# StavrosOrf/EV2Gym

Hardware: AMD Instinct MI355X
Metric: env-steps/sec (envs x chargers x steps); % HBM roofline (higher is better)
Workload: dtype f64; 1 GPU; cfg2: V2GProfitPlusLoads, 50 chargers, 1 transformer, uniform[-1,1] actions; envs_per_gpu=4096, scenario_pool_per_gpu=32768, scenario_pool_order=sorted by busy window inside every window of envs_per_gpu scenarios, chargers=50, transformers=1, steps_per_episode=112, obs_dim=162, soc_log=True, launch=persistent, actor=none

## Files before the change

### ev2gym_amd/csrc/ev2g_device.h

```cpp
#pragma once
#include <hip/hip_runtime.h>
#include <stdint.h>

#define EV2G_BLOCK 256
#define EV2G_NQ 8

struct __attribute__((aligned(128))) SessRec {
    double pacmax, ts;
    double tsm, eta_ch;
    double gate_ch;
    double B;
    double rB;
    double v;
    double rv;
    double gate_dis;
    double minB, emerg;
    double pdismax, eta_dis;
    double cap0;
    double potc;
};
struct SessTail {
    double des;
    int nt_arr, nt_dep;
};
// ... 825 lines not shown
            }
        }
        t += 1;
        __syncthreads();
    }
}

__global__ void ev2g_build_window_table_kernel(DevScn s, double *__restrict__ tab, int m0, int m1) {
    const long long per = (long long)s.R * (s.T + 1) * 40, n = per * m1;
    for (long long i = per * m0 + blockIdx.x * (long long)blockDim.x + threadIdx.x; i < n; i += (long long)gridDim.x * blockDim.x) {
        const int j = (int)(i % 40);
        const long long k = i / 40;
        const int step = (int)(k % (s.T + 1));
        const int er = (int)(k / (s.T + 1));
        tab[i] = (j < 20) ? load_minus_pv_at(s, (long long)er * s.T, step, j) : power_limit_at(s, er, step, j - 20);
    }
}

__global__ void ev2g_build_head_table_kernel(const double *__restrict__ price_ch, const double *__restrict__ win_tab,
                                             int m0, int m1, int T, int NH, double *__restrict__ tab) {
    const long long per = (long long)(T + 1) * NH, n = per * m1;
    for (long long i = per * m0 + blockIdx.x * (long long)blockDim.x + threadIdx.x; i < n; i += (long long)gridDim.x * blockDim.x) {
        const int c = (int)(i % NH);
        const long long row = i / NH;
        const int step = (int)(row % (T + 1));
        const long long e = row / (T + 1);
        double v;
        if (c < 20) { const int k = step + c; v = (k < T) ? fabs(price_ch[e * T + k]) : 0.0; }
        else v = win_tab[row * 40 + (c - 20)];
        tab[i] = v;
    }
}

__global__ void ev2g_build_step_table_kernel(DevScn s, double *__restrict__ tab, int m0, int m1) {
    const long long n = (long long)m1 * s.T;
    for (long long i = (long long)m0 * s.T + blockIdx.x * (long long)blockDim.x + threadIdx.x; i < n; i += (long long)gridDim.x * blockDim.x) {
        double *o = tab + i * 8;
        o[0] = s.price_ch[i]; o[1] = s.price_dis[i]; o[2] = s.tr_base[i]; o[3] = s.tr_maxp[i]; o[4] = s.tr_minp[i];
        o[5] = s.setpoint[i]; o[6] = 0.0; o[7] = 0.0;
    }
}

__global__ void __launch_bounds__(64) ev2g_build_occ_mask_kernel(DevScn s, double *__restrict__ step_tab, int m0, int m1) {
    const int lane = threadIdx.x, P = s.P, T = s.T;
    for (int m = m0 + blockIdx.x; m < m1; m += gridDim.x) {
        int ta = EV2G_INT_MAX, td = -1, ss = -1;
        if (lane < P) {
            const long long gs = (long long)m * P + lane;
            const int2 w = s.port_first_win[gs];
            ta = w.x; td = w.y; ss = s.port_first[gs];
        }
        for (int t = 0; t < T; t++) {
            const bool occ = (ta <= t) && (t <= td);
            if (occ && t >= td) {
                const SessTail tl = s.tail[ss];
                ta = tl.nt_arr; td = tl.nt_dep;
                ss = (ta != EV2G_INT_MAX) ? ss + 1 : -1;
            }
            const unsigned long long m_occ = __ballot(occ), m_arr = __ballot(ta == t + 1);
            if (lane == 0) {
                double *o = step_tab + ((long long)m * T + t) * 8;
                o[6] = __longlong_as_double((long long)m_occ); o[7] = __longlong_as_double((long long)m_arr);
            }
        }
    }
}

__host__ __device__ inline double ev2g_u01(uint64_t seed, uint64_t i) {
    uint64_t z = seed + 0x9E3779B97F4A7C15ull * (i + 1);
    z = (z ^ (z >> 30)) * 0xBF58476D1CE4E5B9ull;
    z = (z ^ (z >> 27)) * 0x94D049BB133111EBull;
    z = z ^ (z >> 31);
    return (double)(z >> 11) * (1.0 / 9007199254740992.0);
}

__global__ void ev2g_fill_uniform_kernel(double *dst, long long n, uint64_t seed, double lo, double hi) {
    for (long long i = blockIdx.x * (long long)blockDim.x + threadIdx.x; i < n; i += (long long)gridDim.x * blockDim.x)
        dst[i] = lo + (hi - lo) * ev2g_u01(seed, (uint64_t)i);
}

__device__ __forceinline__ double wave_sum(double v) {
    for (int d = 32; d > 0; d >>= 1) v += __shfl_xor(v, d, 64);
    return v;
}
__device__ __forceinline__ double wave_min(double v) {
    for (int d = 32; d > 0; d >>= 1) v = fmin(v, __shfl_xor(v, d, 64));
    return v;
}

__device__ __forceinline__ void port_sessions(const DevScn &s, const DevState &st, long long g, long long gs, int cur_step, int &first,
                                              int &last, bool &attached) {
    first = s.port_first[gs];
    last = first;
    attached = false;
    if (first < 0) return;
    const int2 w = make_int2(st.line[g].ta, st.line[g].td);
    const int cur = st.line[g].ss;
    if (cur < 0) {
        last = s.port_end[gs];
    } else {
        attached = (w.x <= cur_step);
        last = attached ? cur + 1 : cur;
    }
}

template <int EPWS> __device__ __forceinline__ double seg_sum(double v) {
    v += xor1_f64(v);
    v += xor2_f64(v);
    v += xor4_f64(v);
    v += dpp_mov_f64<0x128>(v);
    const int lo = __double2loint(v), hi = __double2hiint(v);
    const double r0 = __hiloint2double(__builtin_amdgcn_readlane(hi, 0), __builtin_amdgcn_readlane(lo, 0));
    const double r1 = __hiloint2double(__builtin_amdgcn_readlane(hi, 16), __builtin_amdgcn_readlane(lo, 16));
    const double r2 = __hiloint2double(__builtin_amdgcn_readlane(hi, 32), __builtin_amdgcn_readlane(lo, 32));
    const double r3 = __hiloint2double(__builtin_amdgcn_readlane(hi, 48), __builtin_amdgcn_readlane(lo, 48));
    if (EPWS == 1) return (r0 + r1) + (r2 + r3);
    return (threadIdx.x < 32) ? r0 + r1 : r2 + r3;
}
template <int EPWS> __device__ __forceinline__ double seg_min(double v) {
    v = fmin(v, xor1_f64(v));
    v = fmin(v, xor2_f64(v));
    v = fmin(v, xor4_f64(v));
    v = fmin(v, dpp_mov_f64<0x128>(v));
    const int lo = __double2loint(v), hi = __double2hiint(v);
    const double r0 = __hiloint2double(__builtin_amdgcn_readlane(hi, 0), __builtin_amdgcn_readlane(lo, 0));
    const double r1 = __hiloint2double(__builtin_amdgcn_readlane(hi, 16), __builtin_amdgcn_readlane(lo, 16));
    const double r2 = __hiloint2double(__builtin_amdgcn_readlane(hi, 32), __builtin_amdgcn_readlane(lo, 32));
    const double r3 = __hiloint2double(__builtin_amdgcn_readlane(hi, 48), __builtin_amdgcn_readlane(lo, 48));
    if (EPWS == 1) return fmin(fmin(r0, r1), fmin(r2, r3));
    return (threadIdx.x < 32) ? fmin(r0, r1) : fmin(r2, r3);
}
template <int EPWS> __device__ __forceinline__ bool seg_all(bool p) {
    const unsigned long long m = __ballot(p);
    if (EPWS == 1) return m == ~0ull;
    return (threadIdx.x < 32) ? ((unsigned)m == 0xffffffffu) : ((unsigned)(m >> 32) == 0xffffffffu);
}

struct StatsView {
    int T, C, R, P, dt;
    const double *setpoint;
    const int *scn_sess, *scn_sess_end, *ss_slot, *ss_tarr, *ss_tdep;
    const double *ss_B, *ss_afap;
    const int *cs_served;
    const double *cs_sat_sum, *hist, *env_acc, *sess_final_cap, *sess_abs_e, *soc_log;
    const PortLine *line;
};
__device__ __forceinline__ StatsView ev2g_stats_view(const DevScn &s, const DevState &st, const double *ss_afap) {
    return StatsView{s.T, s.C, s.R, s.P, s.dt, s.setpoint, s.scn_sess, s.scn_sess_end, s.ss_slot, s.ss_tarr, s.ss_tdep, s.ss_B, ss_afap,
                     st.cs_served, st.cs_sat_sum, st.hist, st.env_acc, st.sess_final_cap, st.sess_abs_e, st.soc_log, st.line};
}

#define EV2G_STATS_NK 40
#define EV2G_STATS_TB 8
#define EV2G_STATS_LK 16

template <int EPWS, int NK, int LK>
__device__ __forceinline__ void ev2g_env_stats(const StatsView &sv, int e, bool e_valid, int scn, int lane, int cur_step, double *__restrict__ out,
                                               double *l_keep, int lslot) {
    constexpr int W = 64 / EPWS;
    const int T = sv.T, C = sv.C, R = sv.R, P = sv.P;
    double served = 0.0, sat = 0.0, nsat = 0.0;
    for (int c = lane; c < C; c += W) {
        const int n = sv.cs_served[(long long)e * C + c];
        served += n;
        if (n > 0) { sat += sv.cs_sat_sum[(long long)e * C + c] / n; nsat += 1.0; }
    }
    served = seg_sum<EPWS>(served); sat = seg_sum<EPWS>(sat); nsat = seg_sum<EPWS>(nsat);
    double over = 0.0, te = 0.0, ete = 0.0, ptv = 0.0;
    for (int t = lane; t < T; t += W) {
        const bool past = t < cur_step;
        if (past) for (int r = 0; r < R; r++) over += sv.hist[EV2G_HIST(e, t, T, R) + 2 + r];
        const double sp = sv.setpoint[(long long)scn * T + t], u = past ? sv.hist[EV2G_HIST(e, t, T, R)] : 0.0;
        const double d = sp - u;
        te += d * d;
        ete += fabs(d);
        if (u > sp) ptv += u - sp;
    }
    over = seg_sum<EPWS>(over); te = seg_sum<EPWS>(te); ete = seg_sum<EPWS>(ete); ptv = seg_sum<EPWS>(ptv);
    ete *= (double)sv.dt / 60.0;
    if (lane == 0 && e_valid) {
        double *o = out + (long long)e * 17;
        o[0] = served;
        o[4] = (nsat > 0.0) ? sat / nsat : NAN;
        o[5] = ptv;
        o[6] = te;
        o[7] = ete;
        o[12] = over;
    }
    const double e0 = 7.543e6, e1 = 23.75e6, e2 = 6976, z0 = 7.348e-3, z1 = 3.667, z2 = 7.6e-4, z3 = 4.081e-3;
    const double b_cap_ah = 2.05, b_cap_kwh = 78, d_dist = 15000, b_age = 2 * 365, G_ = 0.186;
    const double theta = 298.15, kk = 0.8263, v_min = 3.3324;
    const double k_arrh = exp(-e2 / theta), k_age = pow(b_age, 0.25);
    const double Q_acc = 2 * (b_age * (d_dist / 365) * G_ * b_cap_ah) / b_cap_kwh, k_qacc = pow(Q_acc, 0.5);
    const bool log_soc = sv.soc_log != nullptr;
    double sum = 0.0, mn = INFINITY, cnt = 0.0, deg_cal = 0.0, deg_cyc = 0.0;
    double vkeep[2];
    int nkeep = 0;
    const int d0 = sv.scn_sess[scn], d1 = sv.scn_sess_end[scn];
    for (int k0 = d0; k0 < d1; k0 += W) {
        const int k = min(k0 + lane, d1 - 1);
        const bool has = k0 + lane < d1;
        const int q = sv.ss_slot[k], ta = sv.ss_tarr[k], td = sv.ss_tdep[k];
        const double B = sv.ss_B[k], afap = sv.ss_afap[k], fin_cap = sv.sess_final_cap[k];
        const double fin_abs = log_soc ? sv.sess_abs_e[k] : 0.0;
        const long long g = (long long)e * P + q;
        const bool spawned = has && ta <= cur_step;
        const bool live = td >= cur_step;
        const double l_cap = sv.line[g].cap, l_abs = sv.line[g].abse;
        const double capk = live ? l_cap : fin_cap;
        if (spawned) {
            const double v = capk / afap * 100.0;
            sum += v;
            mn = fmin(mn, v);
            cnt += 1.0;
            if (nkeep < 2) vkeep[nkeep] = v;
            nkeep++;
        }
        if (spawned) {
            if (log_soc) {
                const double *__restrict__ slog = sv.soc_log + (long long)e * T * P + q;
                const int tend = min(td, cur_step - 1);
                const double soc_f = capk / B;
                const double invB = 1.0 / B;
                double hs = 0.0, fs = 0.0;
                int n = 0, nf = 0;
                double xk[NK];
#pragma unroll
                for (int u = 0; u < NK; u++) xk[u] = slog[(long long)min(ta + u, tend) * P];
#pragma unroll
                for (int u = 0; u < NK; u++) {
                    if (ta + u <= tend) {
                        const double soc = fabs(xk[u]) * invB;
                        hs += soc; n++;
                        if (__double_as_longlong(xk[u]) >= 0) { fs += soc; nf++; }
                    }
                }
                for (int t = ta + NK; t <= tend; t += EV2G_STATS_TB) {
                    double x[EV2G_STATS_TB];
#pragma unroll
                    for (int u = 0; u < EV2G_STATS_TB; u++) x[u] = slog[(long long)min(t + u, tend) * P];
                    if (LK > 0 && t - ta - NK < LK) {
#pragma unroll
                        for (int u = 0; u < EV2G_STATS_TB; u++) l_keep[(t - ta - NK + u) * 64 + lslot] = x[u];
                    }
#pragma unroll
                    for (int u = 0; u < EV2G_STATS_TB; u++) {
                        if (t + u <= tend) {
                            const double soc = fabs(x[u]) * invB;
                            hs += soc; n++;
                            if (__double_as_longlong(x[u]) >= 0) { fs += soc; nf++; }
                        }
                    }
                }
                hs += soc_f; n++;
                fs += soc_f; nf++;
                const double avg_soc = hs / n, avg_f = fs / nf;
                double mad = 0.0;
#pragma unroll
                for (int u = 0; u < NK; u++)
                    if (ta + u <= tend && __double_as_longlong(xk[u]) >= 0) mad += fabs(avg_f - fabs(xk[u]) * invB);
                for (int t = ta + NK; t <= tend; t += EV2G_STATS_TB) {
                    double x[EV2G_STATS_TB];
                    if (LK > 0 && t - ta - NK < LK) {
#pragma unroll
                        for (int u = 0; u < EV2G_STATS_TB; u++) x[u] = l_keep[(t - ta - NK + u) * 64 + lslot];
                    } else {
#pragma unroll
                        for (int u = 0; u < EV2G_STATS_TB; u++) x[u] = slog[(long long)min(t + u, tend) * P];
                    }
#pragma unroll
                    for (int u = 0; u < EV2G_STATS_TB; u++)
                        if (t + u <= tend && __double_as_longlong(x[u]) >= 0) mad += fabs(avg_f - fabs(x[u]) * invB);
                }
                mad += fabs(avg_f - soc_f);
                const double delta_DoD = 2 * (mad / nf);
                const double T_sim = (td - ta + 1) * (double)sv.dt / (60 * 24);
                const double v_avg = v_min + kk * avg_soc;
                const double alpha = (e0 * v_avg - e1) * k_arrh;
                deg_cal += alpha * 0.75 * T_sim / k_age;
                const double v_half = v_min + kk * 0.5;
                const double beta = z0 * (v_half - z1) * (v_half - z1) + z2 + z3 * delta_DoD;
                const double abs_e = live ? l_abs : fin_abs;
                const double Q_sim = (abs_e / b_cap_kwh) * b_cap_ah;
                deg_cyc += beta * 0.5 * Q_sim / k_qacc;
            }
        }
    }
    sum = seg_sum<EPWS>(sum); cnt = seg_sum<EPWS>(cnt); mn = seg_min<EPWS>(mn);
    deg_cal = seg_sum<EPWS>(deg_cal); deg_cyc = seg_sum<EPWS>(deg_cyc);
    if (lane == 0 && e_valid) {
        const double *acc = sv.env_acc + (long long)e * 8;
        double *o = out + (long long)e * 17;
        o[1] = acc[1];
        o[2] = acc[2];
        o[3] = acc[3];
        o[11] = acc[4];
        o[13] = log_soc ? deg_cal + deg_cyc : NAN;
        o[14] = log_soc ? deg_cal : NAN;
        o[15] = log_soc ? deg_cyc : NAN;
        o[16] = acc[0];
    }
    double mean = NAN, sd = NAN, mnv = NAN;
    if (cnt > 0.0) {
        mean = sum / cnt;
        double var = 0.0;
        if (seg_all<EPWS>(nkeep <= 2)) {
            if (nkeep > 0) { const double v = vkeep[0] - mean; var += v * v; }
            if (nkeep > 1) { const double v = vkeep[1] - mean; var += v * v; }
        } else {
            for (int k = d0 + lane; k < d1; k += W) {
                const int ta = sv.ss_tarr[k];
                if (ta <= cur_step) {
                    const double capk = (sv.ss_tdep[k] >= cur_step) ? sv.line[(long long)e * P + sv.ss_slot[k]].cap : sv.sess_final_cap[k];
                    const double v = capk / sv.ss_afap[k] * 100.0 - mean;
                    var += v * v;
                }
            }
        }
        var = seg_sum<EPWS>(var);
        sd = sqrt(var / cnt);
        mnv = mn;
    }
    if (lane == 0 && e_valid) {
        double *o = out + (long long)e * 17;
        o[8] = mean;
        o[9] = sd;
        o[10] = mnv;
    }
}

template <int W>
__device__ __forceinline__ void ev2g_env_reset(const DevScn &s, const DevState &st, int e, int lane, int reset_off, double *__restrict__ r_obs,
                                               float *__restrict__ r_obs32) {
    const int T = s.T, C = s.C, R = s.R, P = s.P;
    const int scn_n = ev2g_scn(e, reset_off, s.M);
    const bool hfast = s.head_tab != nullptr && s.state_kind != 1 && 2 + s.head_nh <= 2 * W && (r_obs || r_obs32);
    double hrow0 = 0.0, hrow1 = 0.0;
    if (hfast) {
        const double *row = s.head_tab + (long long)scn_n * (T + 1) * s.head_nh;
        hrow0 = row[min(max(lane - 2, 0), s.head_nh - 1)];
        hrow1 = row[min(lane + W - 2, s.head_nh - 1)];
    }
    for (int q = lane; q < P; q += W) {
        const long long g = (long long)e * P + q, gs = (long long)scn_n * P + q;
        const int2 w = s.port_first_win[gs];
        st.line[g].ta = w.x; st.line[g].td = w.y; st.line[g].ss = s.port_first[gs]; st.line[g].cyc_lut = 0;
        st.line[g].cap = 0.0; st.line[g].tot = 0.0; st.line[g].prev = 0.0;
        st.port_energy[g] = 0.0; st.port_current[g] = 0.0;
        if (r_obs) { double *o = r_obs + (long long)e * s.D + s.slot_obs[q]; o[0] = 0.0; o[1] = 0.0; if (s.state_kind == 1) o[2] = 0.0; }
        if (r_obs32) { float *o = r_obs32 + (long long)e * s.D + s.slot_obs[q]; o[0] = 0.f; o[1] = 0.f; if (s.state_kind == 1) o[2] = 0.f; }
    }
    for (int c = lane; c < C; c += W) {
        const long long gc = (long long)e * C + c;
        st.cs_sat_sum[gc] = 0.0; st.cs_served[gc] = 0;
        if (st.cs_profits) { st.cs_profits[gc] = 0.0; st.cs_e_ch[gc] = 0.0; st.cs_e_dis[gc] = 0.0; st.cs_power_now[gc] = 0.0; st.cs_cur_now[gc] = 0.0; }
    }
    for (int i = lane; i < 8; i += W) st.env_acc[(long long)e * 8 + i] = 0.0;
    if (lane == 0) st.hist[EV2G_HIST(e, 0, T, R) + 1] = 0.0;
    for (int r = lane; r < R; r += W) st.tr_power_now[(long long)e * R + r] = 0.0;
    if (lane == 0) st.env_fault[e] = 0;
    if (hfast) {
        const int c0 = lane, c1 = lane + W, nc = 2 + s.head_nh;
        const double v0 = (c0 < 2) ? 0.0 : hrow0;
        if (r_obs) { double *o = r_obs + (long long)e * s.D; if (c0 < nc) o[c0] = v0; if (c1 < nc) o[c1] = hrow1; }
        if (r_obs32) { float *o = r_obs32 + (long long)e * s.D; if (c0 < nc) o[c0] = (float)v0; if (c1 < nc) o[c1] = (float)hrow1; }
    } else {
        if (r_obs) write_obs_env(s, r_obs + (long long)e * s.D, scn_n, 0, 0.0, lane, W);
        if (r_obs32) write_obs_env(s, r_obs32 + (long long)e * s.D, scn_n, 0, 0.0, lane, W);
    }
}
// ... 28 lines not shown
```

### ev2gym_amd/csrc/ev2g_step_wave.h

```cpp
#pragma once
#include <type_traits>
#include "ev2g_step_v2.h"
#include "ev2g_mlp.h"

#define EV2G_WAVE_BLOCK 256

__host__ __device__ inline size_t ev2g_wave_lds_bytes(int envs_per_group, int block = EV2G_WAVE_BLOCK) {
    const size_t NS = (size_t)block;
    return sizeof(double) * (EV2G_NQ * (NS + 8) + 7 * NS + 7 * (size_t)envs_per_group + 4 * 64) + sizeof(int) * (6 * NS + 8);
}
#define EV2G_INL_STATS_NK 12
#define EV2G_INL_STATS_LK 16
__host__ __device__ inline size_t ev2g_inl_stats_lds_bytes(int block = EV2G_WAVE_BLOCK) { return (size_t)block * EV2G_INL_STATS_LK * sizeof(double); }
#define EV2G_FUSED_BLOCK 1024
#define EV2G_FUSED_SX 200
#define EV2G_FUSED_RING 10
#define EV2G_FUSED_RING2 7

#define EV2G_FUSED_SXF 196
#define EV2G_FUSED_RINGF 4
__host__ __device__ inline size_t ev2g_fused_lds_bytes(int envs_per_wave = 1, int weight_terms = 1) {
    if (weight_terms > 1)
        return ev2g_wave_lds_bytes(EV2G_FUSED_BLOCK / 64 * envs_per_wave, EV2G_FUSED_BLOCK) + (size_t)16 * EV2G_FUSED_SXF * 4;
    return ev2g_wave_lds_bytes(EV2G_FUSED_BLOCK / 64 * envs_per_wave, EV2G_FUSED_BLOCK) + (size_t)16 * EV2G_FUSED_SX * 2 + (size_t)(25 + 19 + 4) * 16 * 4;
}
struct FusedArgs {
    MlpDev m;
    const float *obs0;
};

typedef const char __attribute__((address_space(1))) *gcptr;
typedef char __attribute__((address_space(1))) *gptr;
template <class T, class B> __device__ __forceinline__ T ldg32(B base, unsigned boff) {
    return *(const T __attribute__((address_space(1))) *)((gcptr)base + boff);
}
template <class T, class B> __device__ __forceinline__ T ldg32_nt(B base, unsigned boff) {
    return __builtin_nontemporal_load((const T __attribute__((address_space(1))) *)((gcptr)base + boff));
}
template <class T, class B> __device__ __forceinline__ void stg32(B base, unsigned boff, T v) {
    *(T __attribute__((address_space(1))) *)((gptr)base + boff) = v;
}
template <class T, class B> __device__ __forceinline__ void stg32_nt(B base, unsigned boff, T v) {
    __builtin_nontemporal_store(v, (T __attribute__((address_space(1))) *)((gptr)base + boff));
}
typedef double d2v __attribute__((ext_vector_type(2)));
typedef double d2v_a8 __attribute__((ext_vector_type(2), aligned(8)));
typedef int i2v __attribute__((ext_vector_type(2)));
typedef int i4v __attribute__((ext_vector_type(4)));
typedef float f2v __attribute__((ext_vector_type(2)));
template <class B> __device__ __forceinline__ SessRec ldg32_rec_charge(B base, unsigned boff) {
    union { SessRec r; d2v v[sizeof(SessRec) / 16]; } u;
    static_assert(sizeof(SessRec) == 128 && offsetof(SessRec, rB) == 48 && offsetof(SessRec, rv) == 64 && offsetof(SessRec, minB) == 80 && offsetof(SessRec, cap0) == 112,
                  "charging reads chunks 0..4, discharging chunks 3..6");
#pragma unroll
    for (int i = 0; i < 5; i++) u.v[i] = ldg32<d2v>(base, boff + 16u * i);
    asm volatile("" : "+v"(u.v[0]), "+v"(u.v[1]), "+v"(u.v[2]), "+v"(u.v[3]), "+v"(u.v[4]));
    return u.r;
}
template <class B> __device__ __forceinline__ SessRec ldg32_rec_discharge(B base, unsigned boff) {
    union { SessRec r; d2v v[sizeof(SessRec) / 16]; } u;
#pragma unroll
    for (int i = 3; i < 7; i++) u.v[i] = ldg32<d2v>(base, boff + 16u * i);
    asm volatile("" : "+v"(u.v[3]), "+v"(u.v[4]), "+v"(u.v[5]), "+v"(u.v[6]));
    return u.r;
}

template <class B> __device__ __forceinline__ SessRec ldg32_cls_charge(B base, unsigned boff) {
    static_assert(sizeof(ClsRec) == 128 && offsetof(ClsRec, gate_ch) == 16 && offsetof(ClsRec, rB) == 32 && offsetof(ClsRec, rv) == 48 && offsetof(ClsRec, v_d) == 64 &&
                  offsetof(ClsRec, gate_dis) == 80 && offsetof(ClsRec, emerg) == 96, "ClsRec layout");
    d2v c[4];
#pragma unroll
    for (int i = 0; i < 4; i++) c[i] = ldg32<d2v>(base, boff + 16u * i);
    asm volatile("" : "+v"(c[0]), "+v"(c[1]), "+v"(c[2]), "+v"(c[3]));
    SessRec r;
    r.pacmax = c[0].x; r.tsm = c[0].y; r.gate_ch = c[1].x; r.B = c[1].y; r.rB = c[2].x; r.v = c[2].y; r.rv = c[3].x;
    return r;
}
template <class B> __device__ __forceinline__ SessRec ldg32_cls_discharge(B base, unsigned boff) {
    d2v c[3];
#pragma unroll
    for (int i = 0; i < 3; i++) c[i] = ldg32<d2v>(base, boff + 64u + 16u * i);
    asm volatile("" : "+v"(c[0]), "+v"(c[1]), "+v"(c[2]));
    SessRec r;
    r.v = c[0].x; r.rv = c[0].y; r.gate_dis = c[1].x; r.minB = c[1].y; r.emerg = c[2].x; r.pdismax = c[2].y;
    return r;
}

struct WaveArgs {
    int P, T, E, D, M;
    char *slab_port; unsigned long long slab_port_slice;
    double *hist;
    double *env_acc;
    const double *cs_pack;
    char *lines;
    const double *step_tab;
    char *port_dyn;
    int dict;
    int epw, es;
};

template <int SK, int RK, bool IO32, int FULLK = 0, int BLOCK = EV2G_WAVE_BLOCK, bool ACT = false, int AE = 1, int NWF = 1>
__global__ void __launch_bounds__(BLOCK, 4) ev2g_step_wave(const V2P *__restrict__ params, StepIO io, int t0,
                                                           int k_steps, int auto_reset, WaveArgs wa, FusedArgs fa) {
    extern __shared__ double lds[];
    static_assert(!ACT || (IO32 && FULLK == 2 && BLOCK == EV2G_FUSED_BLOCK), "the fused actor + step instantiation");
    static_assert(AE == 1 || (ACT && SK == 1 && AE == 2), "two envs per wavefront in the fused instantiation: PublicPST only");
    static_assert(NWF == 1 || (ACT && AE == 1 && NWF == 2), "the float32 policy inside the launch: one env per wavefront (16 policy rows per workgroup)");
    constexpr bool FULL = FULLK >= 1, WIDE = FULLK >= 2, STR = FULLK >= 3 || ACT;
    constexpr bool STR_NT = FULLK >= 3;
    constexpr bool F64 = FULL && !IO32, F32 = FULL && IO32;
    constexpr bool LSO = FULL && !STR;
    constexpr bool INL = FULLK == 2 && !IO32 && !ACT && BLOCK == EV2G_WAVE_BLOCK;
#if defined(EV2G_PHASE_TIMING) && defined(EV2G_PT_OUTER)
    const unsigned long long pt_k0 = __builtin_readcyclecounter();
#endif
    typedef const V2P __attribute__((address_space(4))) *ParamPtr;
    ParamPtr S = (ParamPtr)(unsigned long long)params;
    constexpr int NS = BLOCK;
    constexpr int RS = NS + 8;
    const int P = wa.P, T = wa.T, E = wa.E, D = wa.D, M = wa.M;
    int off = io.scn_off;
    const gptr slabP = (gptr)wa.slab_port, hist = (gptr)wa.hist, slabS = (gptr)S->slab_sess;
    const unsigned long long PS8 = wa.slab_port_slice, SS8 = S->sess_slice;
    const gptr env_acc = (gptr)wa.env_acc;
#define PA(k) (slabP + PS8 * (unsigned long long)(k))
    const int EPW = ACT ? AE : wa.epw;
    const int ES = ACT ? (AE == 1 ? P : 32) : wa.es;
    const int G = (BLOCK / 64) * EPW;
    int grp;
    {
        const int nb = gridDim.x, b = blockIdx.x, per = nb >> 3;
        grp = (nb & 7) == 0 ? (b & 7) * per + (b >> 3) : b;
    }
    const int e0 = grp * G;
    double *stage = lds;
    double *s_cap = stage + (size_t)EV2G_NQ * RS;
    double *s_tot = s_cap + NS, *s_prev = s_tot + NS, *s_bcap = s_prev + NS, *s_potc = s_bcap + NS;
    double *s_amps = s_potc + NS, *s_abse = s_amps + NS;
    double *eacc = s_abse + NS;
    double *s_cst = eacc + 7 * G;
    int *s_ta = (int *)(s_cst + 4 * 64);
    int *s_td = s_ta + NS, *s_ss = s_td + NS, *s_cyc = s_ss + NS, *s_dirty = s_cyc + NS, *items = s_dirty + NS;
    int *cnt = items + NS;
    double *s_ts = s_bcap, *s_etac = s_potc, *s_etad = (double *)s_ta;
    constexpr int LUTMASK = FULL ? 0xfff : 0xffff;
    typedef typename std::conditional<SK == 1, MlpS16<2, 25, 19, 2, 1, 4, AE>, MlpS16<6, 25, 19, 4, 1, 4, AE>>::type MC;
    constexpr int FSX = MC::SX;
    constexpr int FKS1 = (SK == 1) ? 2 : 6, FNT3 = (SK == 1) ? 2 : 4;
    uint16_t *bufX = (uint16_t *)(cnt + 8);
    float *lbias = (float *)(bufX + 16 * EV2G_FUSED_SX);
    float *act_lds = (float *)s_amps;
    uint16_t *bufH1 = (uint16_t *)stage, *bufH2 = bufH1 + 16 * AE * MC::SH1;
    constexpr int FSXF = EV2G_FUSED_SXF;
    float *bufXf = (float *)(cnt + 8);
    static_assert(NWF == 1 || (3 * 16 * MC::SH1 * 2 <= 5 * RS * 8 && EV2G_NQ == 8 && FKS1 * 32 <= 256), "the input rows' bf16 terms live in staging rows 5..7, behind H1's three copies");
    static_assert(NWF == 1 || (FKS1 * 32 + 4 <= FSXF && (3 * MC::SH1 + 2 * MC::SH2) * 16 * 2 <= EV2G_NQ * (EV2G_FUSED_BLOCK + 8) * 8 && MC::SH2 * 16 * 2 <= 16 * FSXF * 4), "float32 policy buffers");
    static_assert(AE * MC::SX <= EV2G_FUSED_SX && MC::NB <= (25 + 19 + 4) * 16 && 16 * AE * (MC::SH1 + MC::SH2) * 2 <= EV2G_NQ * (EV2G_FUSED_BLOCK + 8) * 8, "policy buffers");
    constexpr int ACT_AS = (AE == 1) ? 128 : 64;
    const int tid = threadIdx.x, wv = tid >> 6, lane = tid & 63;
    const bool log_soc = WIDE ? true : (S->soc_log != nullptr);
    const bool log_cs = FULL ? false : (S->cs_profits != nullptr);
    const double dtd = (double)S->dt, sixty_over_dt = S->sixty_over_dt, dt_over_60 = S->dt_over_60;
    const bool pow2_dt = S->pow2_dt != 0;

    const int elw = lane / ES;
    const int q = (ACT && AE == 1) ? lane : lane - elw * ES;
// ... 545 lines not shown
#pragma unroll
            for (int kq = 0; kq < EV2G_NQ - 1; kq++) esum[kq] = stage[kq * RS + (tid_l - q_l)];
        }
        }

        PT_MARK(4)
        const double usage = esum[0];
        const double pf_base = pf_tr.x, pf_maxp = pf_tr.y;
        const double pf_minp = dpp_mov_f64<0x130>(pf_tr.x), pf_sp = dpp_mov_f64<0x130>(pf_tr.y);
        const double tr_power = pf_base + usage;
        const double over = (tr_power > pf_maxp + 0.0001 || tr_power < pf_minp - 0.0001) ? fabs(tr_power - pf_maxp) : 0.0;
        if (WIDE || P >= 3) {
            const double over_n = dpp_mov_f64<0x138>(over);
            if (valid && q_l < 3 && (q_l != 2 || sstep < T)) {
                const double hv = (q_l == 0) ? usage : ((q_l == 1) ? over_n : esum[3]);
                const unsigned hword = (q_l == 0) ? 0u : ((q_l == 1) ? 16u : 32u);
                stg32<double>(hist + (long long)t * 24, (unsigned)(e_l * T) * 24u + hword, hv);
            }
        }
        if (head) {
            double *ea = eacc + elg * 7;
            const double ea0 = ea[0], ea1 = ea[1], ea2 = ea[2], ea3 = ea[3], ea4 = ea[4], ea5 = ea[5];
            const double ea6 = (RK == 3) ? ea[6] : 0.0;
            const unsigned e8 = (unsigned)e_l * 8u;
            double over100 = 0.0;
            if (RK == 0 || RK == 3) over100 = 100.0 * over;
            if (last_step) stg32<double>(S->tr_power_now, e8, tr_power);
            const double potn = esum[3];
            if (!WIDE && P < 3) {
                const unsigned h8 = (unsigned)(e_l * T + t) * 24u;
                stg32<double>(hist, h8 + 16u, over);
                stg32<double>(hist, h8, usage);
                if (sstep < T) stg32<double>(hist, h8 + 32u, potn);
            }
            const double costs = esum[1];
            double reward;
            if (RK == 1) {
                const double pp = ea5;
                const double m = (pp < pf_sp) ? pp : pf_sp;
                const double d = m - usage;
                reward = -(d * d);
            } else if (RK == 2) {
                reward = costs - esum[2];
            } else if (RK == 3) {
                RewardIn ri;
                ri.costs = costs; ri.usage = usage; ri.usage_seq = (S->reward_kind == 4) ? useq : usage; ri.sp = pf_sp; ri.pot_t = ea5; ri.pot_tm1 = ea6; ri.over100 = over100;
                ri.user = esum[2]; ri.tr0_maxp = pf_maxp;
                reward = ev2g_reward(S->reward_kind, ri);
            } else {
                reward = costs - over100 - esum[2];
            }
            const double n0 = ea0 + reward, n1 = ea1 + costs, n2 = ea2 + esum[4], n3 = ea3 + esum[5], n4 = ea4 + esum[6];
            ea[0] = n0; ea[1] = n1; ea[2] = n2; ea[3] = n3; ea[4] = n4; ea[5] = potn;
            if (RK == 3) ea[6] = ea5;
            if (FULL && out) { stg32<double>(rew_run, e8, reward); stg32<uint8_t>(done_run, (unsigned)e_l, (sstep >= T) ? 1 : 0); }
            if (!FULL && io.reward) stg32<double>(io.reward + (long long)kk * io.r_stride, e8, reward);
            if (!FULL && io.done) stg32<uint8_t>(io.done + (long long)kk * io.d_stride, (unsigned)e_l, (sstep >= T) ? 1 : 0);
            if (!FULL && S->x_cost)
                stg32<double>(S->x_cost + (long long)(io.step0 + kk) * S->x_c_stride, e8, (S->cost_kind == 2) ? costs : 100.0 * over + esum[2]);
            if (sstep >= T || last_step) {
                const unsigned a8 = (unsigned)e_l * 64u;
                stg32<d2v>(env_acc, a8, (d2v){n0, n1});
                stg32<d2v>(env_acc, a8 + 16u, (d2v){n2, n3});
                stg32<double>(env_acc, a8 + 32u, n4);
            }
        }
        if ((valid || hcopy) && ((F32 && out) || (!FULL && obs32))) {
            const unsigned o4 = FULL ? hb_obs_env : (unsigned)(e_l * D) * 4u;
            if (SK == 1) {
                if (q_l == 0) {
                    const float h0 = (float)((double)sstep / (double)T), h1 = (float)((sstep < T) ? pf_ob0 : 0.0), h2 = (float)usage;
                    stg32<float>(obs32, o4, h0);
                    stg32<float>(obs32, o4 + 4u, h1);
                    stg32<float>(obs32, o4 + 8u, h2);
                    if (ACT && NWF > 1) { bufXf[arow * FSXF] = h0; bufXf[arow * FSXF + 1] = h1; bufXf[arow * FSXF + 2] = h2; }
                    else
                    if (ACT) {
                        *(uint32_t *)(bufX + arow * FSX) = ev2g_pack_bf16(h0, h1);
                        bufX[arow * FSX + 2] = (uint16_t)ev2g_pack_bf16(h2, 0.f);
                    }
                }
            } else {
                if (q_l == 0) stg32<f2v>(obs32, o4, (f2v){(float)sstep, (float)usage});
                if (q_l < NPAIR) stg32<f2v>(obs32, o4 + 8u + (unsigned)q_l * 8u, (f2v){(float)pf_h0.x, (float)pf_h0.y});
                if (ACT) {
                    if (q_l == 0) xput2(0, (float)sstep, (float)usage);
                    if (q_l < NPAIR) xput2(2 + 2 * q_l, (float)pf_h0.x, (float)pf_h0.y);
                }
                if (!WIDE) {
                    if (q_l + P < NPAIR) stg32<f2v>(obs32, o4 + 8u + (unsigned)(q_l + P) * 8u, (f2v){(float)pf_h1.x, (float)pf_h1.y});
                    const unsigned h8 = (unsigned)((scn * (T + 1) + sstep) * NHEAD) * 8u;
                    for (int pi = q_l + 2 * P; pi < NPAIR; pi += P) {
                        const d2v hv = ldg32<d2v>(S->head_tab, h8 + (unsigned)pi * 16u);
                        stg32<f2v>(obs32, o4 + 8u + (unsigned)pi * 8u, (f2v){(float)hv.x, (float)hv.y});
                    }
                }
            }
        }
        if (valid && ((F64 && out) || (!FULL && obs))) {
            const unsigned o8 = FULL ? hb_obs_env : (unsigned)(e_l * D) * 8u;
            if (SK == 1) {
                if (q_l == 0) {
                    stg32<double>(obs, o8, (double)sstep / (double)T);
                    stg32<double>(obs, o8 + 8u, (sstep < T) ? pf_ob0 : 0.0);
                    stg32<double>(obs, o8 + 16u, usage);
                }
            } else {
                if (STR_NT) {
                    if (q_l == 0) stg32_nt<d2v>(obs, o8, (d2v){(double)sstep, usage});
                    if (q_l < NPAIR) stg32_nt<d2v>(obs, o8 + 16u + (unsigned)q_l * 16u, pf_h0);
                } else {
                if (q_l == 0) stg32<d2v>(obs, o8, (d2v){(double)sstep, usage});
                if (q_l < NPAIR) stg32<d2v>(obs, o8 + 16u + (unsigned)q_l * 16u, pf_h0);
                }
                if (!WIDE) {
                    if (q_l + P < NPAIR) stg32<d2v>(obs, o8 + 16u + (unsigned)(q_l + P) * 16u, pf_h1);
                    const unsigned h8 = (unsigned)((scn * (T + 1) + sstep) * NHEAD) * 8u;
                    for (int pi = q_l + 2 * P; pi < NPAIR; pi += P)
                        stg32<d2v>(obs, o8 + 16u + (unsigned)pi * 16u, ldg32<d2v>(S->head_tab, h8 + (unsigned)pi * 16u));
                }
            }
        }
        PT_MARK(5)
        PT_STEP_END(cntk[0] + cntk[1] == 0)
        t += 1;
        if (STR) { obs_run += io.o_stride; rew_run += io.r_stride; done_run += io.d_stride; mask_run += io.m_stride; }
        if (ACT) obs32_run += io.o_stride;
    }
    __syncthreads();
    if (valid) {
        const int d = s_dirty[tid];
        const unsigned g8 = (unsigned)g * 8u;
        if (d & 3) stg32<i4v>(wa.lines, l64, (i4v){FULL ? r_ta : s_ta[tid], FULL ? r_td : s_td[tid], s_ss[tid], ev2g_line_pack(s_cyc[tid], ((d >> 8) & LUTMASK) - 1)});
        if (d & 1) {
            stg32<d2v>(wa.lines, l64 + 16u, (d2v){s_cap[tid], s_tot[tid]});
            stg32<d2v>(wa.lines, l64 + 32u, (d2v){s_prev[tid], s_abse[tid]});
        }
    }
#if defined(EV2G_PHASE_TIMING) && defined(EV2G_PT_OUTER)
    asm volatile("s_waitcnt vmcnt(0)" ::: "memory");
    PT_MARK(6)
#endif
    PT_FLUSH
    double *stats_out = (INL && t == T && k_steps > 1) ? (double *)S->stats_inl : nullptr;
    if (stats_out != nullptr) {
        __syncthreads();
        const int es = e0 + wv;
        if (es < S->E) {
            const int scn_s = (int)(__builtin_amdgcn_readfirstlane(hb_step) / (64u * (unsigned)T));
            StatsView v{T, S->C, S->R, P, S->dt, (const double *)S->setpoint, (const int *)S->scn_sess, (const int *)S->scn_sess_end,
                        (const int *)S->ss_slot, (const int *)S->ss_tarr, (const int *)S->ss_tdep, (const double *)S->ss_B, (const double *)S->ss_afap,
                        (const int *)S->cs_served, (const double *)S->cs_sat_sum, (const double *)S->hist, (const double *)S->env_acc,
                        (const double *)S->sess_final_cap, (const double *)S->sess_abs_e, (const double *)S->soc_log, (const PortLine *)S->line};
            ev2g_env_stats<1, EV2G_INL_STATS_NK, EV2G_INL_STATS_LK>(v, es, true, scn_s, lane, T, stats_out,
                                                                  lds + (size_t)wv * EV2G_INL_STATS_LK * 64, lane);
        }
    }
}
```

Before: 1.180 billion env-steps/s.

## Use idle wavefront lanes as helper loaders for long session SoC logs in inline stats

In the inline end-of-episode stats, lanes with no session to process now prefetch extra NK-sized chunks of the SoC log for lanes whose sessions are long. Work is assigned with ballot and prefix sums into an LDS map, and the loaded values are staged in per-wave LDS so the owning lanes read them instead of looping serially over global memory. The first-chunk width grows from 12 to 16 and the LDS layout changes to per-wave NK×HC storage. The aim is to shorten the serial tail of the longest session per wave, at the cost of more LDS, extra shuffles and wavefront fences, and higher code complexity.

```diff
diff --git a/ev2gym_amd/csrc/ev2g_device.h b/ev2gym_amd/csrc/ev2g_device.h
--- a/ev2gym_amd/csrc/ev2g_device.h
+++ b/ev2gym_amd/csrc/ev2g_device.h
@@ -1001,9 +1001,10 @@
 
 #define EV2G_STATS_NK 40
 #define EV2G_STATS_TB 8
+#define EV2G_STATS_MC 6
 #define EV2G_STATS_LK 16
 
-template <int EPWS, int NK, int LK>
+template <int EPWS, int NK, int LK, int HC = 0>
 __device__ __forceinline__ void ev2g_env_stats(const StatsView &sv, int e, bool e_valid, int scn, int lane, int cur_step, double *__restrict__ out,
                                                double *l_keep, int lslot) {
     constexpr int W = 64 / EPWS;
@@ -1056,6 +1057,40 @@
         const bool spawned = has && ta <= cur_step;
         const bool live = td >= cur_step;
         const double l_cap = sv.line[g].cap, l_abs = sv.line[g].abse;
+        static_assert(HC == 0 || (EPWS == 1 && LK == 0 && HC <= 64 && EV2G_STATS_MC <= 8), "idle lanes as loaders: one env per wavefront, no parked tail; hcols holds eight bits per chunk");
+        typedef const double __attribute__((address_space(1))) *glog;
+        const char __attribute__((address_space(1))) *sbase = nullptr;
+        int *l_map = (int *)(l_keep + NK * HC);
+        const int tend_h = min(td, cur_step - 1);
+        const int nown = min(d1 - k0, W), nidle = W - nown;
+        int nh = 0, granted = 0, hidx0 = 0;
+        bool helper0 = false;
+        unsigned long long hcols = 0ull;
+        double xk[HC > 0 ? NK : 1];
+        if (HC > 0 && log_soc) {
+            sbase = (const char __attribute__((address_space(1))) *)(sv.soc_log + (long long)__builtin_amdgcn_readfirstlane(e) * T * P);
+            const int len = spawned ? tend_h - ta + 1 : 0;
+            const int extra = (len > NK) ? (len - 1) / NK : 0;
+            const int ncol = nidle > 0 ? HC : 0;
+            const unsigned long long lt = (1ull << lane) - 1ull;
+            int cum = 0;
+#pragma unroll
+            for (int c = 1; c <= EV2G_STATS_MC; c++) {
+                const unsigned long long m = __ballot(extra >= c);
+                const int h = cum + __popcll(m & lt);
+                if (extra >= c && h < ncol) { l_map[h] = lane | (c << 8); granted = c; hcols |= (unsigned long long)h << (8 * (c - 1)); }
+                cum += __popcll(m);
+            }
+            nh = min(cum, ncol);
+            __builtin_amdgcn_fence(__ATOMIC_SEQ_CST, "wavefront");
+            hidx0 = lane - nown;
+            helper0 = hidx0 >= 0 && hidx0 < nh;
+            int src = lane, cc = 0;
+            if (helper0) { const int w = l_map[hidx0]; src = w & 255; cc = w >> 8; }
+            const int tb = __shfl(ta, src, 64) + cc * NK, te_l = __shfl(tend_h, src, 64), q_l = __shfl(q, src, 64);
+#pragma unroll
+            for (int u = 0; u < NK; u++) xk[u] = *(glog)(sbase + (unsigned)(max(min(tb + u, te_l), 0) * P + q_l) * 8u);
+        }
         const double capk = live ? l_cap : fin_cap;
         if (spawned) {
             const double v = capk / afap * 100.0;
@@ -1065,6 +1100,115 @@
             if (nkeep < 2) vkeep[nkeep] = v;
             nkeep++;
         }
+        if (HC > 0) {
+            if (log_soc) {
+                const int tend = tend_h;
+                {
+                    const int hidx = hidx0;
+                    const bool helper = helper0;
+                    if (helper) {
+#pragma unroll
+                        for (int u = 0; u < NK; u++) l_keep[u * HC + hidx] = xk[u];
+                    }
+                }
+                for (int r0 = nidle; r0 < nh; r0 += nidle) {
+                    const int hidx = r0 + lane - nown;
+                    const bool helper = lane >= nown && hidx < nh;
+                    int src = lane, cc = 0;
+                    if (helper) { const int w = l_map[hidx]; src = w & 255; cc = w >> 8; }
+                    const int tb = __shfl(ta, src, 64) + cc * NK, te_l = __shfl(tend, src, 64), q_l = __shfl(q, src, 64);
+                    if (helper) {
+#pragma unroll
+                        for (int u = 0; u < NK; u++) xk[u] = *(glog)(sbase + (unsigned)(max(min(tb + u, te_l), 0) * P + q_l) * 8u);
+#pragma unroll
+                        for (int u = 0; u < NK; u++) l_keep[u * HC + hidx] = xk[u];
+                    }
+                }
+                __builtin_amdgcn_fence(__ATOMIC_SEQ_CST, "wavefront");
+                if (spawned) {
+                    const double *__restrict__ slog = sv.soc_log + (long long)e * T * P + q;
+                    const double soc_f = capk / B;
+                    const double invB = 1.0 / B;
+                    double hs = 0.0, fs = 0.0;
+                    int n = 0, nf = 0;
+#pragma unroll
+                    for (int u = 0; u < NK; u++) {
+                        if (ta + u <= tend) {
+                            const double soc = fabs(xk[u]) * invB;
+                            hs += soc; n++;
+                            if (__double_as_longlong(xk[u]) >= 0) { fs += soc; nf++; }
+                        }
+                    }
+                    static_assert(NK % EV2G_STATS_TB == 0, "chunks are read back in batches of EV2G_STATS_TB");
+#pragma unroll 1
+                    for (int i = 0; i < granted * (NK / EV2G_STATS_TB); i++) {
+                        const int c = i / (NK / EV2G_STATS_TB), u0 = (i % (NK / EV2G_STATS_TB)) * EV2G_STATS_TB, t = ta + (c + 1) * NK + u0;
+                        const double *col = l_keep + u0 * HC + (int)((hcols >> (8 * c)) & 255ull);
+                        double x[EV2G_STATS_TB];
+#pragma unroll
+                        for (int u = 0; u < EV2G_STATS_TB; u++) x[u] = col[u * HC];
+#pragma unroll
+                        for (int u = 0; u < EV2G_STATS_TB; u++) {
+                            if (t + u <= tend) {
+                                const double soc = fabs(x[u]) * invB;
+                                hs += soc; n++;
+                                if (__double_as_longlong(x[u]) >= 0) { fs += soc; nf++; }
+                            }
+                        }
+                    }
+                    for (int t = ta + (1 + granted) * NK; t <= tend; t += EV2G_STATS_TB) {
+                        double x[EV2G_STATS_TB];
+#pragma unroll
+                        for (int u = 0; u < EV2G_STATS_TB; u++) x[u] = slog[(long long)min(t + u, tend) * P];
+#pragma unroll
+                        for (int u = 0; u < EV2G_STATS_TB; u++) {
+                            if (t + u <= tend) {
+                                const double soc = fabs(x[u]) * invB;
+                                hs += soc; n++;
+                                if (__double_as_longlong(x[u]) >= 0) { fs += soc; nf++; }
+                            }
+                        }
+                    }
+                    hs += soc_f; n++;
+                    fs += soc_f; nf++;
+                    const double avg_soc = hs / n, avg_f = fs / nf;
+                    double mad = 0.0;
+#pragma unroll
+                    for (int u = 0; u < NK; u++)
+                        if (ta + u <= tend && __double_as_longlong(xk[u]) >= 0) mad += fabs(avg_f - fabs(xk[u]) * invB);
+#pragma unroll 1
+                    for (int i = 0; i < granted * (NK / EV2G_STATS_TB); i++) {
+                        const int c = i / (NK / EV2G_STATS_TB), u0 = (i % (NK / EV2G_STATS_TB)) * EV2G_STATS_TB, t = ta + (c + 1) * NK + u0;
+                        const double *col = l_keep + u0 * HC + (int)((hcols >> (8 * c)) & 255ull);
+                        double x[EV2G_STATS_TB];
+#pragma unroll
+                        for (int u = 0; u < EV2G_STATS_TB; u++) x[u] = col[u * HC];
+#pragma unroll
+                        for (int u = 0; u < EV2G_STATS_TB; u++)
+                            if (t + u <= tend && __double_as_longlong(x[u]) >= 0) mad += fabs(avg_f - fabs(x[u]) * invB);
+                    }
+                    for (int t = ta + (1 + granted) * NK; t <= tend; t += EV2G_STATS_TB) {
+                        double x[EV2G_STATS_TB];
+#pragma unroll
+                        for (int u = 0; u < EV2G_STATS_TB; u++) x[u] = slog[(long long)min(t + u, tend) * P];
+#pragma unroll
+                        for (int u = 0; u < EV2G_STATS_TB; u++)
+                            if (t + u <= tend && __double_as_longlong(x[u]) >= 0) mad += fabs(avg_f - fabs(x[u]) * invB);
+                    }
+                    mad += fabs(avg_f - soc_f);
+                    const double delta_DoD = 2 * (mad / nf);
+                    const double T_sim = (td - ta + 1) * (double)sv.dt / (60 * 24);
+                    const double v_avg = v_min + kk * avg_soc;
+                    const double alpha = (e0 * v_avg - e1) * k_arrh;
+                    deg_cal += alpha * 0.75 * T_sim / k_age;
+                    const double v_half = v_min + kk * 0.5;
+                    const double beta = z0 * (v_half - z1) * (v_half - z1) + z2 + z3 * delta_DoD;
+                    const double abs_e = live ? l_abs : fin_abs;
+                    const double Q_sim = (abs_e / b_cap_kwh) * b_cap_ah;
+                    deg_cyc += beta * 0.5 * Q_sim / k_qacc;
+                }
+            }
+        } else
         if (spawned) {
             if (log_soc) {
                 const double *__restrict__ slog = sv.soc_log + (long long)e * T * P + q;
diff --git a/ev2gym_amd/csrc/ev2g_step_wave.h b/ev2gym_amd/csrc/ev2g_step_wave.h
--- a/ev2gym_amd/csrc/ev2g_step_wave.h
+++ b/ev2gym_amd/csrc/ev2g_step_wave.h
@@ -9,9 +9,10 @@
     const size_t NS = (size_t)block;
     return sizeof(double) * (EV2G_NQ * (NS + 8) + 7 * NS + 7 * (size_t)envs_per_group + 4 * 64) + sizeof(int) * (6 * NS + 8);
 }
-#define EV2G_INL_STATS_NK 12
-#define EV2G_INL_STATS_LK 16
-__host__ __device__ inline size_t ev2g_inl_stats_lds_bytes(int block = EV2G_WAVE_BLOCK) { return (size_t)block * EV2G_INL_STATS_LK * sizeof(double); }
+#define EV2G_INL_STATS_NK 16
+#define EV2G_INL_STATS_HC 64
+#define EV2G_INL_STATS_WAVE_DOUBLES (EV2G_INL_STATS_NK * EV2G_INL_STATS_HC + 32)
+__host__ __device__ inline size_t ev2g_inl_stats_lds_bytes(int block = EV2G_WAVE_BLOCK) { return (size_t)(block / 64) * EV2G_INL_STATS_WAVE_DOUBLES * sizeof(double); }
 #define EV2G_FUSED_BLOCK 1024
 #define EV2G_FUSED_SX 200
 #define EV2G_FUSED_RING 10
@@ -863,8 +864,8 @@
                         (const int *)S->ss_slot, (const int *)S->ss_tarr, (const int *)S->ss_tdep, (const double *)S->ss_B, (const double *)S->ss_afap,
                         (const int *)S->cs_served, (const double *)S->cs_sat_sum, (const double *)S->hist, (const double *)S->env_acc,
                         (const double *)S->sess_final_cap, (const double *)S->sess_abs_e, (const double *)S->soc_log, (const PortLine *)S->line};
-            ev2g_env_stats<1, EV2G_INL_STATS_NK, EV2G_INL_STATS_LK>(v, es, true, scn_s, lane, T, stats_out,
-                                                                  lds + (size_t)wv * EV2G_INL_STATS_LK * 64, lane);
+            ev2g_env_stats<1, EV2G_INL_STATS_NK, 0, EV2G_INL_STATS_HC>(v, es, true, scn_s, lane, T, stats_out,
+                                                                     lds + (size_t)wv * EV2G_INL_STATS_WAVE_DOUBLES, lane);
         }
     }
 }
```

New measurement: 1.155 billion env-steps/s. 0.979x the previous value.
